# pymc-devs/nutpie

Measured on AMD Instinct MI355X. Metric: leapfrog steps/sec (all chains), higher is better.
Workload: dtype f64

## Files before the change

### include/nutpie_hip.h

```cpp
#ifndef NUTPIE_HIP_H
#define NUTPIE_HIP_H

#include <stdint.h>

#ifdef __cplusplus
extern "C" {
#endif

#define NPHIP_OK 0
#define NPHIP_ERR (-1)
#define NPHIP_ERR_UNKNOWN_ATTR (-2)
#define NPHIP_ERR_NOT_AVAILABLE (-3)
#define NPHIP_ERR_BAD_VALUE (-4)

#define NPHIP_WAIT_DONE 0
#define NPHIP_WAIT_TIMEOUT 1
#define NPHIP_WAIT_ERROR 2

const char* nphip_last_error(void);
const char* nphip_version(void);
int nphip_device_count(void);

typedef struct nphip_settings nphip_settings_t;

// ... 39 lines not shown

typedef struct nphip_sampler nphip_sampler_t;

typedef struct {
    uint64_t finished_draws;
    uint64_t total_draws;
    uint64_t divergences;
    int32_t tuning;
    int32_t started;
    uint64_t latest_num_steps;
    uint64_t total_num_steps;
    double step_size;
    uint64_t runtime_ms;
} nphip_chain_progress_t;

typedef struct {
    int32_t device;
    int32_t waves_per_chain;
    uint64_t chain_offset;
    uint64_t n_local_chains;
    void* stream;
    int32_t store_draws;
    int32_t evals_per_launch;
    int32_t start_paused;
    int32_t manual;
    void* staging_q;
    void* staging_grad;
    void* staging_logp;
    int32_t no_register_kernel;
    int32_t no_stream_cache;
    int32_t graph_steps;
    int32_t host_groups;
    int32_t host_persist;
    int32_t reserved_;
} nphip_launch_t;

void nphip_launch_defaults(nphip_launch_t*);
int nphip_default_evals_per_launch(uint64_t dim);
uint64_t nphip_abi_struct_size(int which );

nphip_sampler_t* nphip_sampler_create(const nphip_settings_t*, const nphip_model_t*, const nphip_launch_t*);
void nphip_sampler_free(nphip_sampler_t*);
int nphip_sampler_wait(nphip_sampler_t*, int64_t timeout_ms);
int nphip_sampler_step(nphip_sampler_t*, uint64_t n_launches, double* kernel_ms, uint64_t* launches_done);
int nphip_sampler_pause(nphip_sampler_t*);
int nphip_sampler_resume(nphip_sampler_t*);
int nphip_sampler_abort(nphip_sampler_t*);
int nphip_sampler_is_finished(nphip_sampler_t*);
int nphip_sampler_progress(nphip_sampler_t*, uint64_t local_chain, nphip_chain_progress_t* out);
int nphip_sampler_waves_per_chain(const nphip_sampler_t*);
uint64_t nphip_sampler_num_chains(const nphip_sampler_t*);
uint64_t nphip_sampler_dim(const nphip_sampler_t*);
uint64_t nphip_sampler_total_draws(const nphip_sampler_t*);
double nphip_sampler_seconds(const nphip_sampler_t*);
uint64_t nphip_sampler_launches(const nphip_sampler_t*);
enum { NPHIP_HOST_MODE_NONE = 0, NPHIP_HOST_MODE_LAUNCH_PER_EVALUATION = 1, NPHIP_HOST_MODE_GROUPS = 2, NPHIP_HOST_MODE_RESIDENT = 3,
       NPHIP_HOST_MODE_FELL_BACK = 4 };
int nphip_sampler_host_mode(const nphip_sampler_t* s);

int nphip_sampler_finished_draws(nphip_sampler_t*, uint64_t* finished);
int nphip_sampler_copy_stat(nphip_sampler_t*, const char* name, void* host_out, uint64_t nbytes);
int nphip_sampler_copy_expanded(nphip_sampler_t*, void* host_out, uint64_t nbytes);
int64_t nphip_sampler_waiting(nphip_sampler_t*, uint8_t* mask);
int nphip_sampler_resume_at(nphip_sampler_t*, uint64_t n, const uint64_t* local_chains, const double* positions, int on_device);
int nphip_sampler_set_metric(nphip_sampler_t*, uint64_t n, const uint64_t* local_chains, uint64_t k, const double* sigma2, const double* V,
                             const double* lambda, int on_device);
int nphip_sampler_stage_metric(nphip_sampler_t*, uint64_t n, const uint64_t* local_chains, uint64_t k, const double* sigma2, const double* V,
// ... 28 lines not shown
```

### nutpie_amd/_lib.py

```python

from __future__ import annotations

import ctypes as C
import json
import os
import subprocess
import threading

import numpy as np

_HERE = os.path.dirname(os.path.abspath(__file__))
_LIB_PATH = os.environ.get("NUTPIE_HIP_LIB") or os.path.join(_HERE, "libnutpie_hip.so")
_CSRC = os.path.join(_HERE, "csrc")

__version__ = "0.1.0"

NPHIP_OK = 0
NPHIP_ERR_UNKNOWN_ATTR = -2
NPHIP_ERR_NOT_AVAILABLE = -3
NPHIP_ERR_BAD_VALUE = -4
WAIT_DONE, WAIT_TIMEOUT, WAIT_ERROR = 0, 1, 2

RAW_LOGP_FN = C.CFUNCTYPE(C.c_int, C.c_uint64, C.POINTER(C.c_double), C.POINTER(C.c_double), C.POINTER(C.c_double), C.c_void_p)
RAW_EXPAND_FN = C.CFUNCTYPE(C.c_int, C.c_uint64, C.c_uint64, C.POINTER(C.c_double), C.POINTER(C.c_double), C.c_void_p)
DEVICE_EXPAND_FN = C.CFUNCTYPE(C.c_int, C.c_uint64, C.c_uint64, C.c_uint64, C.c_void_p, C.c_void_p, C.c_void_p, C.c_void_p)
DEVICE_LOGP_FN = C.CFUNCTYPE(C.c_int, C.c_uint64, C.c_uint64, C.c_void_p, C.c_void_p, C.c_void_p, C.c_void_p, C.c_void_p)


class _Launch(C.Structure):
    _fields_ = [
        ("device", C.c_int32),
        ("waves_per_chain", C.c_int32),
        ("chain_offset", C.c_uint64),
        ("n_local_chains", C.c_uint64),
        ("stream", C.c_void_p),
        ("store_draws", C.c_int32),
        ("evals_per_launch", C.c_int32),
        ("start_paused", C.c_int32),
        ("manual", C.c_int32),
        ("staging_q", C.c_void_p),
        ("staging_grad", C.c_void_p),
        ("staging_logp", C.c_void_p),
        ("no_register_kernel", C.c_int32),
        ("no_stream_cache", C.c_int32),
        ("graph_steps", C.c_int32),
        ("host_groups", C.c_int32),
        ("host_persist", C.c_int32),
        ("reserved_", C.c_int32),
    ]


class _Progress(C.Structure):
    _fields_ = [
        ("finished_draws", C.c_uint64),
        ("total_draws", C.c_uint64),
        ("divergences", C.c_uint64),
        ("tuning", C.c_int32),
        ("started", C.c_int32),
        ("latest_num_steps", C.c_uint64),
        ("total_num_steps", C.c_uint64),
        ("step_size", C.c_double),
        ("runtime_ms", C.c_uint64),
    ]


_lib = None
_lib_lock = threading.Lock()


def build(force: bool = False) -> str:
    srcs = [os.path.join(_CSRC, f) for f in ("kernels.hip", "host.hip", "linalg.hip", "lowrank_est.hip", "engine_types.h", "kernel_families.h", "dense_tile.h", "Makefile")]
    srcs += [os.path.join(_HERE, "..", "include", f) for f in ("nutpie_hip.h", "nphip_spec.h")]
    stale = not os.path.exists(_LIB_PATH) or os.path.getmtime(_LIB_PATH) < max(os.path.getmtime(s) for s in srcs)
    if force or stale:
        r = subprocess.run(["make", "-j", str(max(1, min(8, os.cpu_count() or 1))), "-C", _CSRC] + (["-B"] if force else []), capture_output=True, text=True)
        if r.returncode != 0:
            raise RuntimeError("building libnutpie_hip.so failed:\n" + r.stdout + r.stderr)
    return _LIB_PATH


def lib():
# ... 469 lines not shown

_STAT_DTYPES = {
    "depth": np.int64, "n_steps": np.int64, "index_in_trajectory": np.int64,
    "diverging": np.bool_, "maxdepth_reached": np.bool_, "tuning": np.bool_,
    "energy": np.float64, "energy_error": np.float64, "logp": np.float64, "step_size": np.float64,
    "step_size_bar": np.float64, "mean_tree_accept": np.float64, "mean_tree_accept_sym": np.float64,
}
_VECTOR_STATS = ("gradient", "mass_matrix_inv", "divergence_start", "divergence_end", "divergence_momentum", "divergence_start_gradient")


class PyTrace:

    def __init__(self, draws, stats, finished, chain_offset=0, expanded=None):
        self.draws = draws
        self.stats = stats
        self.finished = finished
        self.chain_offset = chain_offset
        self.expanded = expanded

    def is_arrow(self):
        return False

    def is_zarr(self):
        return False

    def is_dense(self):
        return True


class PySampler:

    def __init__(self, settings: PyNutsSettings, model: _Model, *, device=0, waves_per_chain=0, chain_offset=0,
                 n_local_chains=0, stream=None, store_draws=True, evals_per_launch=0, start_paused=False, manual=False,
                 staging=None, no_register_kernel=False, no_stream_cache=False, graph_steps=0, host_groups=0, host_persist=None):
        L = lib()
        la = _Launch()
        L.nphip_launch_defaults(C.byref(la))
        la.device = int(device)
        la.waves_per_chain = int(waves_per_chain)
        la.chain_offset = int(chain_offset)
        la.n_local_chains = int(n_local_chains)
        la.stream = C.c_void_p(stream) if stream else None
        la.store_draws = int(bool(store_draws))
        la.evals_per_launch = int(evals_per_launch)
        la.start_paused = int(bool(start_paused))
        la.manual = int(bool(manual))
        la.no_register_kernel = int(bool(no_register_kernel))
        la.no_stream_cache = int(bool(no_stream_cache))
        la.graph_steps = int(graph_steps)
        la.host_groups = int(host_groups)
        if host_persist is None:
            host_persist = 1 if getattr(model, "_python_callable", False) else 0
        la.host_persist = int(host_persist)
        if staging is not None:
            la.staging_q, la.staging_grad, la.staging_logp = (C.c_void_p(int(p)) for p in staging)
        self._model = model
        self._settings = settings
        self._chain_offset = int(chain_offset)
        self._store_draws = bool(store_draws)
        h = L.nphip_sampler_create(settings._h, model._h, C.byref(la))
        if not h:
            raise RuntimeError(_err())
        self._h = C.c_void_p(h)
        self._results = None

    @classmethod
    def from_pyfunc(cls, settings, cores, model, progress_type=None, extra_callback=None, extra_callback_rate=None, store=None, **kw):
        if store is not None:
            raise NotImplementedError("storage back-ends (zarr / arrow) are outside the scope of the HIP engine: the trace lives in HBM")
        if progress_type is not None or extra_callback is not None:
            raise NotImplementedError("progress templates / callbacks are handled by nutpie_amd.sample(), not by the sampler handle")
        return cls(settings, model, **kw)

    from_pymc = from_pyfunc
    from_stan = from_pyfunc

    def _require(self):
        if self._h is None:
            raise RuntimeError("Sampler is empty (results were taken)")

    @property
# ... 333 lines not shown
```

### nutpie_amd/csrc/engine_types.h

```cpp
#pragma once

#include <stdint.h>

namespace nphip {

constexpr int kMaxDepthCap = 16;
constexpr int kLrMax = 16;

enum Phase : int64_t {
    PH_START = 0,
    PH_INIT_EVAL = 1,
    PH_SS_FIRST = 2,
    PH_SS_ITER = 3,
    PH_TREE = 4,
    PH_DONE = 5,
    PH_ERROR = 6,
    PH_WAIT_HOST = 7,
    PH_RESUME_SS = 8,
    PH_DRAW_END = 9,
    PH_DRAW_BEGIN = 10,
};

enum ChainError : int64_t {
    CE_NONE = 0,
// ... 79 lines not shown
struct Args {
    DevSettings s;
    int64_t n_chains;
    int64_t chain_offset;
    int64_t dim, ld;
    int32_t cap;
    int32_t npslots, nqpool;
    Ctl* ctl;
    double* qpool;
    double* pslots;
    double* sig2;
    double* est;
    const double* m_mu;
    const double* m_a;
    const double* m_b;
    const double* m_bsh;
    double* qeval;
    double* geval;
    double* ueval;
    int64_t* ecode;
    const double* init_points;
    double* tr_draws;
    double* tr_grad;
    double* tr_mm;
    double* tr_div[4];
    int64_t* st_depth; int64_t* st_nsteps; int64_t* st_idx;
    uint8_t* st_diverging; uint8_t* st_maxdepth; uint8_t* st_tuning;
    double* st_energy; double* st_energy_error; double* st_logp; double* st_step; double* st_step_bar;
    double* st_accept; double* st_accept_sym;
    int32_t reg_nv;
    int32_t stream_cache;
    int32_t sig_lds;
    int32_t lean;
    int32_t max_evals;
    int32_t have_result;
    unsigned long long* counters;
    unsigned int* grp_arrive;
    volatile unsigned long long* grp_flag;
    volatile unsigned long long* grp_go;
    unsigned long long* grp_go_dev;
    int32_t pvec;
    int32_t lr_on;
    float* lr_V;
    double* lr_lam;
    double* lr_std;
    double* st_sig2;
    float* st_V;
    double* st_lam;
    const void* dens_data;
    int32_t dens_lds_doubles;
    int32_t dens_shared_doubles;
    const double* dg_P;
    const double* dg_mu;
    int64_t dg_KP;
    unsigned long long* dg_sync;
    int32_t dg_variant, dg_pad_;
};
constexpr int kDgSyncWords = 128 * 32 + 16 + 16 + 8 * 256 / 2;
constexpr unsigned long long kGoLast = 1ull << 32;
constexpr unsigned long long kGoSeqMask = 0xffffffffull;
constexpr unsigned long long kPubAllDone = 1ull << 62, kPubError = 1ull << 63;
constexpr unsigned long long kRollGo = 1, kRollFail = 2;

struct LaunchSlice {
    int chain_lo, chain_n;
    int grp;
// ... 10 lines not shown
```

### nutpie_amd/csrc/host.hip

```cpp
#include <hip/hip_runtime.h>
#include <sched.h>

#include <algorithm>
#include <atomic>
#include <chrono>
#include <cmath>
#include <condition_variable>
#include <cstdio>
#include <cstring>
#include <functional>
#include <memory>
#include <map>
#include <mutex>
#include <string>
#include <thread>
#include <vector>

#include "../../include/nutpie_hip.h"
#include "../../include/nphip_spec.h"
#include "engine_types.h"
#include "kernel_families.h"

namespace nphip {
hipError_t launch_advance(const Args& a, const Args* d_args, bool fused, int W, hipStream_t st, const LaunchSlice* slice = nullptr);
// ... 811 lines not shown
    s.early_mm_switch_freq = (int64_t)set.early_mass_matrix_switch_freq;
    s.mm_update_freq = (int64_t)set.mass_matrix_update_freq;
    s.initial_step = set.initial_step; s.target_accept = set.target_accept;
    s.jitter = set.jitter; s.max_step_size = set.max_step_size;
    s.adapt_adam = set.adam ? 1 : 0; s.adam_lr = set.adam_learning_rate;
    s.da_k = set.da_k; s.da_t0 = set.da_t0; s.da_gamma = set.da_gamma;
    s.init_kind = model.init_kind; s.num_try_init = (int32_t)set.num_try_init;
    s.store_draws = launch.store_draws; s.store_gradient = set.store_gradient;
    s.store_mass_matrix = set.store_mass_matrix; s.store_divergences = set.store_divergences;
    if (!set.pause_draws.empty()) {
        if (!launch.manual) { set_error("pause draws need a manual-mode sampler (launch.manual = 1): the caller resumes the chains"); return false; }
        for (uint64_t pd : set.pause_draws)
            if (pd == 0 || pd >= set.num_tune) { set_error("pause draws must lie inside the warm-up (0 < draw < num_tune)"); return false; }
    }
    s.n_pause = (int32_t)set.pause_draws.size();
    for (size_t i = 0; i < set.pause_draws.size(); ++i) s.pause_draws[i] = (int64_t)set.pause_draws[i];

    args.n_chains = (int64_t)n;
    args.chain_offset = (int64_t)launch.chain_offset;
    args.dim = (int64_t)dim;
    args.ld = geo.ld;
    args.cap = (int32_t)set.maxdepth;
    args.npslots = num_pslots(args.cap);
    args.nqpool = num_qpool(args.cap);
    const size_t ld = (size_t)args.ld;
    args.reg_nv = geo.reg_nv;
    args.lean = geo.lean ? 1 : 0;
    args.stream_cache = geo.stream_cache ? 1 : 0;
    args.pvec = lrm ? 3 : 2;
    args.lr_on = lrm ? 1 : 0;
    s.low_rank_metric = lrm ? 1 : 0;

    args.sig_lds = geo.sig_lds ? 1 : 0;

    if (!dalloc(&args.ctl, n)) return false;
    if (!dalloc(&args.qpool, n * args.nqpool * 2 * ld)) return false;
    if (!dalloc(&args.pslots, n * args.npslots * (size_t)args.pvec * ld)) return false;
    if (lrm && (!dalloc(&args.lr_V, n * (size_t)kLrMax * ld) || !dalloc(&args.lr_lam, n * (size_t)kLrMax) || !dalloc(&args.lr_std, n * ld))) return false;
    if (lrm && (!dalloc(&args.st_V, n * (size_t)kLrMax * ld) || !dalloc(&args.st_lam, n * (size_t)kLrMax) || !dalloc(&args.st_sig2, n * ld))) return false;
    if (!dalloc(&args.sig2, n * ld)) return false;
    if (!dalloc(&args.est, n * 8 * ld)) return false;
    if (!dalloc(&args.counters, 4)) return false;
    if (fused) {
        double *mu = nullptr, *a = nullptr, *b = nullptr;
        if (!dalloc(&mu, ld) || !dalloc(&a, ld) || !dalloc(&b, ld)) return false;
        HIP_TRY(hipMemcpyAsync(mu, model.mu.data(), dim * 8, hipMemcpyHostToDevice, stream));
        HIP_TRY(hipMemcpyAsync(a, model.a.data(), dim * 8, hipMemcpyHostToDevice, stream));
        bpad.assign(ld, -0.0);
        std::copy(model.b.begin(), model.b.begin() + (dim > 0 ? dim - 1 : 0), bpad.begin());
        HIP_TRY(hipMemcpyAsync(b, bpad.data(), ld * 8, hipMemcpyHostToDevice, stream));
        args.m_mu = mu; args.m_a = a; args.m_b = b;
        double* bsh = nullptr;
        if (!dalloc(&bsh, ld + 8)) return false;
        bshpad.assign(ld + 8, -0.0);
        std::copy(model.b.begin(), model.b.begin() + (dim > 0 ? dim - 1 : 0), bshpad.begin() + 1);
        HIP_TRY(hipMemcpyAsync(bsh, bshpad.data(), (ld + 8) * 8, hipMemcpyHostToDevice, stream));
        args.m_bsh = bsh;
    } else {
        const uint64_t zc_limit = (n <= 1024 && dim <= 1024) ? (8u << 20) : (4u << 20);
        zero_copy = (model.kind == 1) && !(launch.staging_q && launch.staging_grad && launch.staging_logp) && n * dim * 8 <= zc_limit;
        if (launch.staging_q && launch.staging_grad && launch.staging_logp) {
            args.qeval = (double*)launch.staging_q; args.geval = (double*)launch.staging_grad; args.ueval = (double*)launch.staging_logp;
        } else if (!zero_copy && (!dalloc(&args.qeval, n * dim) || !dalloc(&args.geval, n * dim) || !dalloc(&args.ueval, n))) return false;
        if (dens) {
            args.dens_data = model.jit_data;
            args.dens_lds_doubles = (int32_t)(model.jit_lds_bytes / 8);
// ... 1269 lines not shown
```

### nutpie_amd/csrc/kernel_families.h

```cpp
#pragma once
#include <cstddef>
#include <cstdint>
#include <type_traits>
#include <utility>

#ifndef NPHIP_W1_OCC2_MAX
#ifdef NPHIP_JIT_DENSITY
#define NPHIP_W1_OCC2_MAX 0
#else
#define NPHIP_W1_OCC2_MAX 3
#endif
#endif
#ifndef NPHIP_RW_OCC2_MAX
#define NPHIP_RW_OCC2_MAX 4
#endif
#ifndef NPHIP_CB_OCC
#define NPHIP_CB_OCC(W) 2
#endif
#ifndef NPHIP_LEAN_OCC
#define NPHIP_LEAN_OCC(W) ((W) <= 4 ? 1 : ((W) <= 8 ? 2 : 4))
#endif

namespace nphip {

// ... 2 lines not shown

enum class DynLds : int {
    none,
    sigma2,
    sigma2_and_summary,
    sigma2_if_staged
};

struct KernelFamily {
    Family family;
    bool fused, lean, remote, lr, wide, denseg;
    int waves;
    int nv_lo, nv_hi;
    int part;
    DynLds dyn;
};

inline constexpr KernelFamily kW1One         = {Family::w1,             true,  false, false, false, false, false, 1,                  1, 1,   0,    DynLds::none};
inline constexpr KernelFamily kW1            = {Family::w1,             true,  false, false, false, false, false, 1,                  2, 8,   12,   DynLds::none};
inline constexpr KernelFamily kW1Wide        = {Family::w1_wide,        true,  false, false, false, true,  false, 1,                  2, 3,   12,   DynLds::none};
inline constexpr KernelFamily kW1Lr          = {Family::w1_lr,          true,  false, false, true,  false, false, 1,                  1, 8,   8,    DynLds::none};
inline constexpr KernelFamily kRing          = {Family::ring,           true,  false, false, false, false, false, 2 | 4,              1, 8,   3,    DynLds::none};
inline constexpr KernelFamily kRingLr        = {Family::ring_lr,        true,  false, false, true,  false, false, 2 | 4,              5, 8,   9,    DynLds::none};
inline constexpr KernelFamily kLean4         = {Family::lean,           true,  true,  false, false, false, false, 4,                  9, 24,  1,    DynLds::sigma2_and_summary};
inline constexpr KernelFamily kLean8         = {Family::lean,           true,  true,  false, false, false, false, 8,                  1, 10,  2,    DynLds::sigma2};
inline constexpr KernelFamily kMemory        = {Family::memory,         true,  false, false, false, false, false, 1 | 2 | 4 | 8 | 16, -1, 0,  4,    DynLds::sigma2_if_staged};
inline constexpr KernelFamily kMemoryCached  = {Family::memory,         true,  false, false, false, false, false, 1,                  -8, -8, 4,    DynLds::none};
inline constexpr KernelFamily kRemoteW1      = {Family::remote,         false, false, true,  false, false, false, 1,                  1, 8,   5,    DynLds::none};
inline constexpr KernelFamily kRemoteWn      = {Family::remote,         false, false, true,  false, false, false, 2 | 4,              1, 8,   6,    DynLds::none};
inline constexpr KernelFamily kDenseResident = {Family::dense_resident, false, false, true,  false, false, true,  1,                  1, 8,   11,   DynLds::none};

inline constexpr KernelFamily kFamilies[] = {kW1One, kW1, kW1Wide, kW1Lr, kRing, kRingLr, kLean4, kLean8, kMemory, kMemoryCached, kRemoteW1, kRemoteWn, kDenseResident};

inline constexpr int kWideMaxChains = 1024;
inline constexpr int kMemoryWaves = 8;
inline constexpr int kMaxWaves = 16;

constexpr bool has(const KernelFamily& f, int W, int64_t nv) { return W > 0 && (f.waves & W) == W && (W & (W - 1)) == 0 && nv >= f.nv_lo && nv <= f.nv_hi; }
constexpr int chains_per_group(int W) { return W == 1 ? 4 : 1; }
constexpr int group_threads(int W) { return 64 * W * chains_per_group(W); }

inline constexpr int kLdsBytes = 160 * 1024, kChunkBytes = 128 * 8;
constexpr int lean_free_chunks(int W, int nv) { return W == 4 ? (kLdsBytes - (nv > 20 ? 12288 : 8192) - nv * W * kChunkBytes) / (W * kChunkBytes) : 0; }

constexpr size_t dyn_lds_bytes(const KernelFamily& f, int W, int nv, int64_t ld, bool sig_lds) {
    const size_t sigma2 = (size_t)ld * 8;
    const int free_chunks = lean_free_chunks(W, nv), summary = free_chunks < 0 ? 0 : (free_chunks < 2 * nv ? free_chunks : 2 * nv);
    return f.dyn == DynLds::sigma2 ? sigma2
         : f.dyn == DynLds::sigma2_and_summary ? sigma2 + (size_t)summary * (size_t)(W * kChunkBytes)
         : (f.dyn == DynLds::sigma2_if_staged && W >= 8 && sig_lds) ? sigma2 : 0;
}

constexpr bool two_waves_per_simd(int W, int NV, bool LR, bool WIDE) { return NV > 0 && !LR && !WIDE && NV <= (W == 1 ? NPHIP_W1_OCC2_MAX : NPHIP_RW_OCC2_MAX); }
template <bool FUSED, int W, int NV, bool LEAN, bool REMOTE, bool LR, bool WIDE>
constexpr int min_waves() { return LEAN ? NPHIP_LEAN_OCC(W) : (two_waves_per_simd(W, NV, LR, WIDE) ? 2 : ((!FUSED && NV == 0 && !REMOTE) ? NPHIP_CB_OCC(W) : 1)); }
template <bool FUSED, int W, int NV, bool LEAN, bool REMOTE, bool LR, bool WIDE>
constexpr int max_waves() { return LEAN ? NPHIP_LEAN_OCC(W) : (two_waves_per_simd(W, NV, LR, WIDE) ? 2 : 8); }

#ifdef NPHIP_ONLY_FAMILY
#ifndef NPHIP_ONLY_W
#define NPHIP_ONLY_W 0
#endif
#ifndef NPHIP_ONLY_NV
#define NPHIP_ONLY_NV -1000
#endif
constexpr bool built(const KernelFamily& f, int W, int nv) {
// ... 15 lines not shown
```

### nutpie_amd/csrc/kernels.hip

```cpp
#include <hip/hip_runtime.h>

#include "../../include/nphip_spec.h"
#include "engine_types.h"
#include "kernel_families.h"

#if defined(__HIP_DEVICE_COMPILE__)
#define NPHIP_GLOBAL __attribute__((address_space(1)))
#define NPHIP_LDS __attribute__((address_space(3)))
#define NPHIP_CONST __attribute__((address_space(4)))
#else
#define NPHIP_GLOBAL
#define NPHIP_LDS
#define NPHIP_CONST
#endif

#ifdef NPHIP_JIT_DENSITY
#define NPHIP_JIT 1
#else
#define NPHIP_JIT 0
#endif

namespace nphip {


// ... 1808 lines not shown
    __device__ __forceinline__ void issue_leaf_hot(Hot& H) const {
        const int32_t j = H.nleaf + 1, d = H.depth;
        int32_t newp;
        if (j == (1 << d)) newp = H.end_newp;
        else if (j & 1) newp = (j == 1) ? slot_first(d) : slot_first(__builtin_ctz((unsigned)(j - 1)));
        else newp = slot_last(__builtin_ctz((unsigned)j), A.cap);
        H.newq = (int32_t)__builtin_ctz(~(H.used_base | H.sub_used | (1u << H.srcq)));
        H.newp = newp;
    }
    __device__ __forceinline__ void start_doubling_hot(Hot& H) const {
        nphip_u32x4 r = nphip_philox(A.s.seed, (uint32_t)H.depth, gchain, H.draw, NPHIP_RNG_DIRECTION);
        H.dir = (r.v[0] & 1u) ? 1 : -1;
        const int db = H.dir > 0 ? 1 : 0;
        H.nleaf = 0;
        H.srcq = rfl(c->endq[db]);
        H.srcp = rfl(c->endp[db]);
        H.idx_cur = rfl(H.dir > 0 ? c->idx_right : c->idx_left);
        H.sub_used = 0u;
        hot_doubling(H);
        issue_leaf_hot(H);
    }
    __device__ __forceinline__ double merge_uniform_hot(const Hot& H, int32_t j, int32_t d, int32_t k, nphip_u32x4& blk, int32_t& blk_id) const {
        const int32_t id = k >> 1;
        if (blk_id != id) {
            const uint32_t c3 = (uint32_t)NPHIP_RNG_MERGE | ((uint32_t)d << 8) | ((uint32_t)id << 16);
            blk = nphip_philox(A.s.seed, (uint32_t)j, gchain, H.draw, c3);
            blk_id = id;
        }
        return (k & 1) ? nphip_u01(blk.v[2], blk.v[3]) : nphip_u01(blk.v[0], blk.v[1]);
    }

    __device__ __forceinline__ void merge_level(Hot& H, int32_t j, int32_t d, int32_t k, nphip_u32x4& blk, int32_t& blk_id, double& T_wm, int64_t& T_we,
                                                int32_t& T_q, double& T_U, double& T_E, int32_t& T_idx) {
        double sm; int64_t se;
        const int32_t A_q = rfl(c->sub_q[k]), A_idx = rfl(c->sub_idx[k]);
        const double A_U = c->sub_U[k], A_E = c->sub_E[k];
        H.sub_used &= ~(1u << A_q);
        nphip_w_add(c->sub_wm[k], c->sub_we[k], T_wm, T_we, &sm, &se);
        const bool take = merge_uniform_hot(H, j, d, k, blk, blk_id) * sm < nphip_w_rel(T_wm, T_we, se);
        if (!take) { T_q = A_q; T_U = A_U; T_E = A_E; T_idx = A_idx; }
        T_wm = sm; T_we = se;
    }

    __device__ __forceinline__ bool leaf_reg(RegsT& X, Hot& H, int32_t& end_code_out) {
        constexpr int nk = NVX;
        const int32_t j = H.nleaf + 1, d = H.depth, dir = H.dir;
        const int db = dir > 0 ? 1 : 0;
        const int32_t idx_new = H.idx_cur + dir;
        const int32_t srcq = H.srcq, srcp = H.srcp, newq = H.newq, newp = H.newp;
        const bool check = H.check;
#ifdef NPHIP_PROFILE
        const int64_t tp0 = (int64_t)__builtin_readcyclecounter();
#endif
        if (X.reg_q != srcq) {
            const double* q = Q(srcq);
#pragma unroll
            for (int k = 0; k < NVX; ++k) if (k < nk) X.q[k] = ld2(q, ridx(k));
            if (REMOTE) {
                const double* g = G(srcq);
#pragma unroll
                for (int k = 0; k < NVX; ++k) if (k < nk) X.g[k] = ld2(g, ridx(k));
            } else {
                regs_grad(X);
            }
        }
        if (X.reg_p != srcp) { load_slot(srcp, X.p, X.r); if (LR) load_slot_v(srcp, X.v); }
        if (!X.sig_ok) {
#pragma unroll
            for (int k = 0; k < NVX; ++k) if (k < nk) X.s[k] = ld2(sig2, ridx(k));
            if (LR) {
                const double* sdp = A.lr_std + (size_t)chain * ld;
#pragma unroll
                for (int k = 0; k < NVX; ++k) X.sd[k] = ld2(sdp, ridx(k));
            }
            X.sig_ok = true;
        }
        if (j == 1) { X.ring_leaf0 = -1; X.ring_leaf1 = -1; }
        const bool lrm = LR && lr_job() && rfl(c->host_metric) != 0;
// ... 139 lines not shown
            lr_dispatch(lrk, [&](auto kc) {
#pragma unroll
                for (int k = 0; k < NVX; ++k) {
                    double2 u;
                    u.x = X.sd[k].x * X.p[k].x; u.y = X.sd[k].y * X.p[k].y;
                    const double2 w = lr_apply_c<decltype(kc)::value>(ridx(k), u, lrc);
                    X.v[k].x = X.sd[k].x * w.x; X.v[k].y = X.sd[k].y * w.y;
                }
            });
#pragma unroll
            for (int k = 0; k < NVX; ++k) {
                accK.x = fma(X.p[k].x, X.v[k].x, accK.x);
                accK.y = fma(X.p[k].y, X.v[k].y, accK.y);
                const double tx0 = (X.r[k].x - rold[k].x) + pold[k].x, ty0 = (X.r[k].y - rold[k].y) + pold[k].y;
                accE.x = fma(tx0, X.v[k].x, accE.x);
                accE.y = fma(ty0, X.v[k].y, accE.y);
                accS.x = fma(tx0, vold[k].x, accS.x);
                accS.y = fma(ty0, vold[k].y, accS.y);
            }
        }
        X.reg_q = newq;
        X.reg_p = newp;
        X.dirty_qg = true;
        X.dirty_pr = true;
        if (!LR && !NORING) {
            if ((j & 3) == 1) { ring_write(0, X.p, X.r); X.ring_leaf0 = j; }
            else if ((j & 3) == 2) { ring_write(1, X.p, X.r); X.ring_leaf1 = j; }
        }
#ifdef NPHIP_PROFILE
        const int64_t tp1 = (int64_t)__builtin_readcyclecounter();
#endif
        NPHIP_PHASE_FENCE();
        double v4[4] = {accK.x + accK.y, accL.x + accL.y, accE.x + accE.y, accS.x + accS.y};
        rsum(v4);
        NPHIP_PHASE_FENCE();
#ifdef NPHIP_PROFILE
        const int64_t tp2 = (int64_t)__builtin_readcyclecounter();
        c->prof[0] += tp1 - tp0; c->prof[6] += tp2 - tp1;
#endif
        const double K = 0.5 * v4[0], lp = (REMOTE && !DG) ? lp_remote : 0.5 * v4[1];
        const bool turn0 = (v4[2] < 0.0) || (v4[3] < 0.0);
        if (REMOTE && code_remote < 0) { X.dirty_qg = X.dirty_pr = false; hot_save(H); finish_chain(PH_ERROR, CE_FATAL_LOGP); return true; }
        H.nleaf += 1;
        H.n_steps += 1;
        const bool ok = isfinite(lp) && (!REMOTE || code_remote == 0);
        const double Unew = -lp, E = K + Unew, dE = E - H.H0;
        const bool diverged = !ok || (dE > H.max_ee) || !isfinite(dE);
        double T_wm = 1.0;
        int64_t T_we = 0;
        nphip_u32x4 mrg_blk = {{0u, 0u, 0u, 0u}};
        int32_t mrg_id = -1;
        {
            if (!diverged) {
                const double x = -dE, xc = x > 1e9 ? 1e9 : (x < -1e9 ? -1e9 : x);
                double kk;
                nphip_exp_parts(xc, &T_wm, &kk);
                T_we = (int64_t)kk;
                const double e = nphip_exp_scale(x, T_wm, kk);
                const double a = e < 1.0 ? e : 1.0;
                H.acc += a;
                H.acc_sym += 2.0 * a / (1.0 + e);
            }
        }
        if (diverged) { X.dirty_qg = X.dirty_pr = false; hot_save(H);
            if (ENDOUT) end_code_out = end_code(true, false, FUSED, ok, !REMOTE, FUSED); else rare_end_draw(A, c, red, chain, true, false, FUSED, ok, !REMOTE, FUSED);
            return true; }
#ifdef NPHIP_PROFILE
        int64_t tq = (int64_t)__builtin_readcyclecounter();
        c->prof[8] += tq - tp2;
#endif

        NPHIP_PHASE_FENCE();
        double T_U = Unew, T_E = E;
        int32_t T_q = newq, T_idx = idx_new;
        H.srcq = newq; H.srcp = newp; H.idx_cur = idx_new;
        double2 obp[NVX], obr[NVX], obv[NVX];
        int32_t k = 0;
        while (k < d && (((j - 1) >> k) & 1)) {
            if (check) {
                bool turn;
                if (k == 0) {
                    turn = turn0;
                } else if (LR) {
                    const int32_t a = j - (2 << k) + 1, al = j - (1 << k);
                    load_slot(first_slot_of(a, d), obp, obr); load_slot_v(first_slot_of(a, d), obv);
// ... 3 lines not shown
#pragma unroll
                        for (int q_ = 0; q_ < NVX; ++q_) { pold[q_] = obp[q_]; rold[q_] = obr[q_]; vold[q_] = obv[q_]; }
                    }
                    if (!turn) {
                        const int32_t sl_ = slot_last(__builtin_ctz((unsigned)al), A.cap);
                        load_slot(sl_, obp, obr); load_slot_v(sl_, obv);
                        turn = sub_b_v(X, obp, obr, obv);
                    }
                } else {
                    const int32_t a = j - (2 << k) + 1, al = j - (1 << k);
                    if (k == 1 && X.ring_leaf0 == a) ring_read(0, obp, obr);
                    else load_slot(first_slot_of(a, d), obp, obr);
                    if (k == 2) {
                        if (X.ring_leaf0 == al + 1) ring_read(0, pold, rold);
                        else load_slot(first_slot_of(al + 1, d), pold, rold);
                    }
                    turn = sub_a(X, obp, obr, pold, rold);
                    if (k >= 2) {
#pragma unroll
                        for (int q_ = 0; q_ < NVX; ++q_) { pold[q_] = obp[q_]; rold[q_] = obr[q_]; }
                    }
                    if (!turn) {
                        if (k == 1 && X.ring_leaf1 == al) ring_read(1, obp, obr);
                        else load_slot(slot_last(__builtin_ctz((unsigned)al), A.cap), obp, obr);
                        turn = sub_b(X, obp, obr);
                    }
                }
                if (turn) { X.dirty_qg = X.dirty_pr = false; hot_save(H); if (ENDOUT) end_code_out = end_code(false, false, false, false, !REMOTE, false); else rare_end_draw(A, c, red, chain, false, false, false, false, !REMOTE); return true; }
            }
#ifdef NPHIP_PROFILE
            { const int64_t t_ = (int64_t)__builtin_readcyclecounter(); c->prof[k == 0 ? 9 : 10] += t_ - tq; tq = t_; }
#endif
            NPHIP_PHASE_FENCE();
            merge_level(H, j, d, k, mrg_blk, mrg_id, T_wm, T_we, T_q, T_U, T_E, T_idx);
            NPHIP_PHASE_FENCE();
#ifdef NPHIP_PROFILE
            { const int64_t t_ = (int64_t)__builtin_readcyclecounter(); c->prof[11] += t_ - tq; tq = t_; }
#endif
            ++k;
        }
        if (k < d) {
            c->sub_wm[k] = T_wm; c->sub_we[k] = T_we; c->sub_q[k] = T_q; c->sub_U[k] = T_U; c->sub_E[k] = T_E; c->sub_idx[k] = T_idx;
            H.sub_used |= 1u << T_q;
#ifdef NPHIP_PROFILE
            const int64_t tp3 = (int64_t)__builtin_readcyclecounter();
#endif
            store_state(X, T_q == newq, LR || NORING || ((j & 3) == 0) || ((j & 7) == 1));
            issue_leaf_hot(H);
#ifdef NPHIP_PROFILE
            c->prof[7] += (int64_t)__builtin_readcyclecounter() - tp3;
#endif
            return false;
        }
        bool turn = false;
        if (check) {
            const int32_t far_slot = rfl(c->endp[1 - db]), far_idx = rfl(dir > 0 ? c->idx_left : c->idx_right);
            const int32_t near_idx = rfl(dir > 0 ? c->idx_right : c->idx_left);
            if (d == 0) {
                turn = LR ? check1_v(X, pold, pold, vold, far_idx, idx_new) : check1(X, pold, pold, far_idx, idx_new);
            } else if (LR) {
                if (d == 2) { load_slot(slot_first((int)d), pold, rold); load_slot_v(slot_first((int)d), vold); }
                load_slot(far_slot, obp, obr); load_slot_v(far_slot, obv);
                turn = check_a_v(X, obp, obr, obv, pold, rold, vold, far_idx, near_idx + dir, idx_new);
                if (!turn) {
                    load_slot(rfl(c->endp[db]), obp, obr); load_slot_v(rfl(c->endp[db]), obv);
                    turn = check1_v(X, obp, obr, obv, near_idx, idx_new);
                }
// ... 1202 lines not shown
                    if (budget <= 0) break;
                    --budget;
                } else {
                    if (!have) break;
                    have = false;
                }
            }
            worked = true;
            if (ph != PH_TREE) {
                rare_phase_fn(A, c, red, chain, ph);
                continue;
            }
            RegsT X;
            SCacheT Y;
            Hot H;
            constexpr bool HOT = NV > 0;
            if (HOT) hot_load(H);
            int32_t end_code_ = 0;
            bool rare = false, out_of_budget = false;
            int lean_end = 0;
            const LeanRs lrs = lean_rs();
            if ((NV == 0 || NV == -1 || LEAN) && sig_copy != nullptr) {
                for (int64_t i = 2 * (int64_t)threadIdx.x; i < ld; i += 2 * (int64_t)blockDim.x)
                    *(NPHIP_LDS double2*)(sig_copy + i) = ld2(sig2, i);
                __syncthreads();
                sig_lds = sig_copy;
            }
            for (;;) {
#ifdef NPHIP_PROFILE
                const int64_t t0 = (int64_t)__builtin_readcyclecounter();
#endif
                if (NV > 0) {
                    if (LEAN) { lean_end = leaf_lean(lrs, X, H); rare = lean_end != 0; }
                    else rare = leaf_reg(X, H, end_code_);
                } else {
                    double lp = 0.0;
                    int64_t code = 0;
                    if (FUSED && !lr_job()) {
                        bool turn0 = false;
                        const bool even_leaf = ((c->nleaf + 1) & 1) == 0;
                        const double K = lf_stream(lp, c->idx_cur + c->dir, turn0, Y);
                        rare = cont_tree(X, Y, K, lp, code, even_leaf, turn0);
                    } else {
                        if (FUSED) lf1(c->lf_srcq, c->lf_srcp, c->lf_newq, c->lf_newp, c->lf_sign);
                        CbCrit cr;
                        bool fast = false;
                        if (cb_fast_ok()) {
                            lp = A.ueval[chain];
                            code = A.ecode ? A.ecode[chain] : 0;
                            fast = code == 0 && isfinite(lp);
                        }
                        const double K = fast ? leaf_cb(cr) : lf2(lp, code, c->idx_cur + c->dir);
#ifdef NPHIP_PROFILE
                        c->prof[0] += (int64_t)__builtin_readcyclecounter() - t0;
#endif
                        rare = cont_tree(X, Y, K, lp, code, false, false, fast ? &cr : nullptr);
                    }
                }
#ifdef NPHIP_PROFILE
                const int64_t t2 = (int64_t)__builtin_readcyclecounter();
                c->prof[3] += 1;
                if (rare) { c->prof[2] += t2 - t0; c->prof[5] += 1; } else { c->prof[1] += t2 - t0; c->prof[4] += 1; }
#endif
                if (rare || (!HOT && c->phase != PH_TREE)) break;
                if (REMOTE && !DENS && !DG) {
                    if (c->hs_last != 0) { out_of_budget = true; break; }
                } else if (FUSED || DENS || DG) {
// ... 619 lines not shown
```

### profiles/make_traffic.py

```python
import json
import os
import re

HERE = os.path.dirname(os.path.abspath(__file__))
SOURCES = {
    "1000:1": ("r6_d1000_timed_config_pmc.txt", 1024 * 2048, "k_advance<fused,W=1,NV=8>",
               "bench.py default: sampling phase, positions stored, 2048 leapfrogs per chain per launch; the timed launches"),
    "2000:2": ("r1_d2000_multiwave_kernel_pmc.txt", 1024 * 128, "k_advance<fused,W=2,NV=8>", "round 1: tuning phase, 128 leapfrogs per chain per launch"),
    "10000:4": ("r5_d10000_timed_config_pmc.txt", 1024 * 512, "k_advance<fused,W=4,NV=20,lean>",
                "bench.py --dim 10000: sampling phase, positions stored, 512 leapfrogs per chain per launch; the timed launches"),
}
JOBS = {
    "config3_compiled_density": ("r6_config3_compiled_density_final_pmc.txt", "k_advance<callback,W=1,NV=2,REMOTE> of the generated radon density (512 chains, tune 400 + draws 1000)"),
    "config3_traced_torch_density": ("r6_config3_traced_torch_density_final_pmc.txt", "the same model traced from its torch log-density (nutpie_amd.torch_trace)"),
    "low_rank_173_k4": ("r5_low_rank_d173_k4_pmc.txt", "k_advance<fused,W=1,NV=2,LR>: AR(1) Gaussian D = 173, 512 chains, 4 columns handed in; the launches after the hand-in"),
    "config2ii_dense_resident": ("r6_dense_resident_pmc.txt", "k_advance<callback,W=1,NV=8,REMOTE,DENSEG>: the dense 1000-dim Gaussian's resident kernel (launch-wide fp64 MFMA GEMM inside the leaf), 1024 chains; 12 launches of 256 evaluation rounds in the sampling phase (scratch/r6_dense_job.py)"),
    "low_rank_1000_k16": ("r5_low_rank_d1000_k16_pmc.txt", "k_advance<fused,W=1,NV=8,LR>: AR(1) Gaussian D = 1000, 1024 chains, 16 columns handed in; the launches after the hand-in"),
}
FALLBACK = {
    "1000:1": ("r2_d1000_kernel_pmc.txt", 1024 * 256, "round 2: tuning phase, 256 leapfrogs per chain per launch"),
    "10000:4": ("r2_d10000_lean_lds_slot_e128_pmc.txt", 1024 * 128, "round 2: tuning phase, 128 leapfrogs per chain per launch"),
}


def counter(txt, name):
    m = re.search(name + r"\s+n=\s*\d+\s+mean=([0-9.e+]+)", txt)
    return float(m.group(1)) if m else None


def main():
    out = {}
    for key, (fn, lpl, kernel, config) in SOURCES.items():
        if not os.path.exists(os.path.join(HERE, fn)) and key in FALLBACK:
            fn, lpl, config = FALLBACK[key]
        txt = open(os.path.join(HERE, fn)).read()
        f, w = counter(txt, "FETCH_SIZE"), counter(txt, "WRITE_SIZE")
        e = {"bytes_per_leapfrog": (2 * f + w) * 1024 / lpl, "leapfrogs_per_launch": lpl, "kernel": kernel, "source": "profiles/" + fn,
             "config": config, "fetch_size_kb": f, "write_size_kb": w}
        insts = {k: counter(txt, "SQ_INSTS_" + k.upper()) for k in ("valu", "salu", "lds", "vmem_rd", "vmem_wr")}
# ... 40 lines not shown
```

Baseline: 240.2 million.

## Fuse pairs of leapfrog leaves into one reduction and acceptance pass

Adds a paired-leaf path for single-wave fused kernels with small NV. The first leaf's leapfrog is run inline and its kinetic and log-density partial sums ride along in the second leaf's cross-lane reduction. The two acceptance exponentials are computed in the two wave halves, and the first leaf is merged as a tree record without a separate leaf iteration. This is meant to halve reduction and sync overhead per leaf. It costs register pressure and extra rollback logic when the first leaf diverges. It can be disabled with a new launch flag.

```diff
diff --git a/include/nutpie_hip.h b/include/nutpie_hip.h
--- a/include/nutpie_hip.h
+++ b/include/nutpie_hip.h
@@ -95,7 +95,7 @@
     int32_t graph_steps;
     int32_t host_groups;
     int32_t host_persist;
-    int32_t reserved_;
+    int32_t no_leaf_pairs;
 } nphip_launch_t;
 
 void nphip_launch_defaults(nphip_launch_t*);
diff --git a/nutpie_amd/_lib.py b/nutpie_amd/_lib.py
--- a/nutpie_amd/_lib.py
+++ b/nutpie_amd/_lib.py
@@ -46,7 +46,7 @@
         ("graph_steps", C.c_int32),
         ("host_groups", C.c_int32),
         ("host_persist", C.c_int32),
-        ("reserved_", C.c_int32),
+        ("no_leaf_pairs", C.c_int32),
     ]
 
 
@@ -582,7 +582,8 @@
 
     def __init__(self, settings: PyNutsSettings, model: _Model, *, device=0, waves_per_chain=0, chain_offset=0,
                  n_local_chains=0, stream=None, store_draws=True, evals_per_launch=0, start_paused=False, manual=False,
-                 staging=None, no_register_kernel=False, no_stream_cache=False, graph_steps=0, host_groups=0, host_persist=None):
+                 staging=None, no_register_kernel=False, no_stream_cache=False, graph_steps=0, host_groups=0, host_persist=None,
+                 no_leaf_pairs=False):
         L = lib()
         la = _Launch()
         L.nphip_launch_defaults(C.byref(la))
@@ -597,6 +598,7 @@
         la.manual = int(bool(manual))
         la.no_register_kernel = int(bool(no_register_kernel))
         la.no_stream_cache = int(bool(no_stream_cache))
+        la.no_leaf_pairs = int(bool(no_leaf_pairs))
         la.graph_steps = int(graph_steps)
         la.host_groups = int(host_groups)
         if host_persist is None:
diff --git a/nutpie_amd/csrc/engine_types.h b/nutpie_amd/csrc/engine_types.h
--- a/nutpie_amd/csrc/engine_types.h
+++ b/nutpie_amd/csrc/engine_types.h
@@ -135,6 +135,7 @@
     int32_t stream_cache;
     int32_t sig_lds;
     int32_t lean;
+    int32_t no_leaf_pairs;
     int32_t max_evals;
     int32_t have_result;
     unsigned long long* counters;
diff --git a/nutpie_amd/csrc/host.hip b/nutpie_amd/csrc/host.hip
--- a/nutpie_amd/csrc/host.hip
+++ b/nutpie_amd/csrc/host.hip
@@ -867,6 +867,7 @@
     s.low_rank_metric = lrm ? 1 : 0;
 
     args.sig_lds = geo.sig_lds ? 1 : 0;
+    args.no_leaf_pairs = launch.no_leaf_pairs != 0 ? 1 : 0;
 
     if (!dalloc(&args.ctl, n)) return false;
     if (!dalloc(&args.qpool, n * args.nqpool * 2 * ld)) return false;
diff --git a/nutpie_amd/csrc/kernel_families.h b/nutpie_amd/csrc/kernel_families.h
--- a/nutpie_amd/csrc/kernel_families.h
+++ b/nutpie_amd/csrc/kernel_families.h
@@ -58,6 +58,11 @@
 
 inline constexpr KernelFamily kFamilies[] = {kW1One, kW1, kW1Wide, kW1Lr, kRing, kRingLr, kLean4, kLean8, kMemory, kMemoryCached, kRemoteW1, kRemoteWn, kDenseResident};
 
+#ifndef NPHIP_LEAF_PAIRS_NV_MASK
+#define NPHIP_LEAF_PAIRS_NV_MASK 0x1FC
+#endif
+constexpr bool leaf_pairs(int W, int NV) { return W == 1 && NV >= 2 && NV <= 8 && ((NPHIP_LEAF_PAIRS_NV_MASK >> NV) & 1) != 0; }
+
 inline constexpr int kWideMaxChains = 1024;
 inline constexpr int kMemoryWaves = 8;
 inline constexpr int kMaxWaves = 16;
diff --git a/nutpie_amd/csrc/kernels.hip b/nutpie_amd/csrc/kernels.hip
--- a/nutpie_amd/csrc/kernels.hip
+++ b/nutpie_amd/csrc/kernels.hip
@@ -1864,18 +1864,124 @@
 
     __device__ __forceinline__ void merge_level(Hot& H, int32_t j, int32_t d, int32_t k, nphip_u32x4& blk, int32_t& blk_id, double& T_wm, int64_t& T_we,
                                                 int32_t& T_q, double& T_U, double& T_E, int32_t& T_idx) {
-        double sm; int64_t se;
         const int32_t A_q = rfl(c->sub_q[k]), A_idx = rfl(c->sub_idx[k]);
         const double A_U = c->sub_U[k], A_E = c->sub_E[k];
+        merge_record(H, j, d, k, blk, blk_id, A_q, A_idx, A_U, A_E, c->sub_wm[k], c->sub_we[k], T_wm, T_we, T_q, T_U, T_E, T_idx);
+    }
+    __device__ __forceinline__ void merge_record(Hot& H, int32_t j, int32_t d, int32_t k, nphip_u32x4& blk, int32_t& blk_id, int32_t A_q, int32_t A_idx,
+                                                 double A_U, double A_E, double A_wm, int64_t A_we, double& T_wm, int64_t& T_we,
+                                                 int32_t& T_q, double& T_U, double& T_E, int32_t& T_idx) {
+        double sm; int64_t se;
         H.sub_used &= ~(1u << A_q);
-        nphip_w_add(c->sub_wm[k], c->sub_we[k], T_wm, T_we, &sm, &se);
+        nphip_w_add(A_wm, A_we, T_wm, T_we, &sm, &se);
         const bool take = merge_uniform_hot(H, j, d, k, blk, blk_id) * sm < nphip_w_rel(T_wm, T_we, se);
         if (!take) { T_q = A_q; T_U = A_U; T_E = A_E; T_idx = A_idx; }
         T_wm = sm; T_we = se;
     }
 
-    __device__ __forceinline__ bool leaf_reg(RegsT& X, Hot& H, int32_t& end_code_out) {
+    static constexpr bool PAIRS = FUSED && !LEAN && !REMOTE && !LR && !NORING && nphip::leaf_pairs(W, NV);
+    struct PairA {
+        int32_t nleaf, idx_cur, srcq, srcp, newq, newp;
+        uint32_t sub_used;
+        double accK, accL;
+    };
+    __device__ __forceinline__ void pair_first(RegsT& X, Hot& H, PairA& a) {
         constexpr int nk = NVX;
+        const int32_t j = H.nleaf + 1, dir = H.dir, idx_new = H.idx_cur + dir;
+        a.nleaf = H.nleaf; a.idx_cur = H.idx_cur; a.srcq = H.srcq; a.srcp = H.srcp; a.newq = H.newq; a.newp = H.newp; a.sub_used = H.sub_used;
+#ifdef NPHIP_PROFILE
+        const int64_t tp0 = (int64_t)__builtin_readcyclecounter();
+#endif
+        if (X.reg_q != H.srcq) {
+            const double* q = Q(H.srcq);
+#pragma unroll
+            for (int k = 0; k < NVX; ++k) if (k < nk) X.q[k] = ld2(q, ridx(k));
+            regs_grad(X);
+        }
+        if (X.reg_p != H.srcp) load_slot(H.srcp, X.p, X.r);
+        if (!X.sig_ok) {
+#pragma unroll
+            for (int k = 0; k < NVX; ++k) if (k < nk) X.s[k] = ld2(sig2, ridx(k));
+            X.sig_ok = true;
+        }
+        if (j == 1) { X.ring_leaf0 = -1; X.ring_leaf1 = -1; }
+        NPHIP_PHASE_FENCE();
+        const double eps = (double)dir * H.step;
+        const double h = 0.5 * eps;
+        if (idx_new == -1) {
+#pragma unroll
+            for (int k = 0; k < NVX; ++k) if (k < nk) { X.r[k].x = -0.0; X.r[k].y = -0.0; }
+        }
+        double2 z[NVX];
+#pragma unroll
+        for (int k = 0; k < NVX; ++k) if (k < nk) {
+            X.p[k].x = fma(h, X.g[k].x, X.p[k].x);
+            X.p[k].y = fma(h, X.g[k].y, X.p[k].y);
+            X.q[k].x = fma(eps, X.s[k].x * X.p[k].x, X.q[k].x);
+            X.q[k].y = fma(eps, X.s[k].y * X.p[k].y, X.q[k].y);
+            const double2 mu = par_mu(ridx(k));
+            z[k].x = X.q[k].x - mu.x;
+            z[k].y = X.q[k].y - mu.y;
+        }
+        publish_edges(z);
+        double2 accK = {0.0, 0.0}, accL = {0.0, 0.0};
+#pragma unroll
+        for (int k = 0; k < NVX; ++k) if (k < nk) {
+            double2 aa, b01, gg;
+            double b2, edge_zl, edge_zr;
+            par_ab(ridx(k), aa, b01, b2);
+            edge_pair(z, k, edge_zl, edge_zr);
+            const double zl = wave_shr1(z[k].y, edge_zl);
+            const double zr = wave_shl1(z[k].x, edge_zr);
+            double tx = aa.x * z[k].x;
+            tx = fma(b01.x, zl, tx);
+            tx = fma(b01.y, z[k].y, tx);
+            double ty = aa.y * z[k].y;
+            ty = fma(b01.y, z[k].x, ty);
+            ty = fma(b2, zr, ty);
+            gg.x = -tx;
+            gg.y = -ty;
+            accL.x = fma(z[k].x, gg.x, accL.x);
+            accL.y = fma(z[k].y, gg.y, accL.y);
+            X.g[k] = gg;
+            X.p[k].x = fma(h, gg.x, X.p[k].x);
+            X.p[k].y = fma(h, gg.y, X.p[k].y);
+            X.r[k].x = X.r[k].x + X.p[k].x;
+            X.r[k].y = X.r[k].y + X.p[k].y;
+            accK.x = fma(X.p[k].x, X.s[k].x * X.p[k].x, accK.x);
+            accK.y = fma(X.p[k].y, X.s[k].y * X.p[k].y, accK.y);
+        }
+        a.accK = accK.x + accK.y;
+        a.accL = accL.x + accL.y;
+        X.reg_q = H.newq;
+        X.reg_p = H.newp;
+        X.dirty_qg = true;
+        X.dirty_pr = true;
+        if ((j & 3) == 1) { ring_write(0, X.p, X.r); X.ring_leaf0 = j; }
+        store_state(X, true, (j & 7) == 1);
+        H.nleaf = j;
+        H.n_steps += 1;
+        H.srcq = a.newq; H.srcp = a.newp; H.idx_cur = idx_new;
+        H.sub_used |= 1u << a.newq;
+        issue_leaf_hot(H);
+#ifdef NPHIP_PROFILE
+        c->prof[0] += (int64_t)__builtin_readcyclecounter() - tp0;
+#endif
+    }
+    static __device__ __forceinline__ double exp_scale_select(double x, double p, double k) {
+        const int ki = (int)k;
+        const int k1 = ki / 2, k2 = ki - k1;
+        double e = (p * nphip_pow2i(k1)) * nphip_pow2i(k2);
+        e = x < -745.2 ? 0.0 : e;
+        e = x > 709.782712893384 ? (double)INFINITY : e;
+        return e;
+    }
+
+    __device__ __forceinline__ bool leaf_reg(RegsT& X, Hot& H, int32_t& end_code_out, const bool pair_ = false, bool* a_ended = nullptr) {
+        constexpr int nk = NVX;
+        const bool PAIR = PAIRS && pair_;
+        PairA pa = {};
+        if (PAIR) { pair_first(X, H, pa); NPHIP_PHASE_FENCE(); }
         const int32_t j = H.nleaf + 1, d = H.depth, dir = H.dir;
         const int db = dir > 0 ? 1 : 0;
         const int32_t idx_new = H.idx_cur + dir;
@@ -2081,7 +2187,14 @@
 #endif
         NPHIP_PHASE_FENCE();
         double v4[4] = {accK.x + accK.y, accL.x + accL.y, accE.x + accE.y, accS.x + accS.y};
-        rsum(v4);
+        double vA[2] = {0.0, 0.0};
+        if (PAIR) {
+            double v8[8] = {v4[0], v4[1], v4[2], v4[3], pa.accK, pa.accL, 0.0, 0.0};
+            rsum(v8);
+            v4[0] = v8[0]; v4[1] = v8[1]; v4[2] = v8[2]; v4[3] = v8[3]; vA[0] = v8[4]; vA[1] = v8[5];
+        } else {
+            rsum(v4);
+        }
         NPHIP_PHASE_FENCE();
 #ifdef NPHIP_PROFILE
         const int64_t tp2 = (int64_t)__builtin_readcyclecounter();
@@ -2090,6 +2203,19 @@
         const double K = 0.5 * v4[0], lp = (REMOTE && !DG) ? lp_remote : 0.5 * v4[1];
         const bool turn0 = (v4[2] < 0.0) || (v4[3] < 0.0);
         if (REMOTE && code_remote < 0) { X.dirty_qg = X.dirty_pr = false; hot_save(H); finish_chain(PH_ERROR, CE_FATAL_LOGP); return true; }
+        double A_U = 0.0, A_E = 0.0, A_dE = 0.0;
+        if (PAIR) {
+            const double K_A = 0.5 * vA[0], lp_A = 0.5 * vA[1];
+            const bool ok_A = isfinite(lp_A);
+            A_U = -lp_A; A_E = K_A + A_U; A_dE = A_E - H.H0;
+            if (!ok_A || (A_dE > H.max_ee) || !isfinite(A_dE)) {
+                H.idx_cur = pa.idx_cur; H.srcq = pa.srcq; H.srcp = pa.srcp; H.newq = pa.newq; H.newp = pa.newp; H.sub_used = pa.sub_used;
+                X.dirty_qg = X.dirty_pr = false; hot_save(H);
+                end_code_out = end_code(true, false, FUSED, ok_A, !REMOTE, FUSED);
+                *a_ended = true;
+                return true;
+            }
+        }
         H.nleaf += 1;
         H.n_steps += 1;
         const bool ok = isfinite(lp) && (!REMOTE || code_remote == 0);
@@ -2099,7 +2225,30 @@
         int64_t T_we = 0;
         nphip_u32x4 mrg_blk = {{0u, 0u, 0u, 0u}};
         int32_t mrg_id = -1;
-        {
+        double A_wm = 1.0;
+        int64_t A_we = 0;
+        if constexpr (PAIRS) {
+            if (PAIR || !diverged) {
+            const double x = lane < 32 ? -A_dE : -dE, xc = x > 1e9 ? 1e9 : (x < -1e9 ? -1e9 : x);
+            double wm, kk;
+            nphip_exp_parts(xc, &wm, &kk);
+            const double e = exp_scale_select(x, wm, kk);
+            const double a = e < 1.0 ? e : 1.0;
+            const double sym = 2.0 * a / (1.0 + e);
+            if (PAIR) {
+                A_wm = readlane_f64(wm, 0);
+                A_we = (int64_t)readlane_f64(kk, 0);
+                H.acc += readlane_f64(a, 0);
+                H.acc_sym += readlane_f64(sym, 0);
+            }
+            if (!diverged) {
+                T_wm = readlane_f64(wm, 32);
+                T_we = (int64_t)readlane_f64(kk, 32);
+                H.acc += readlane_f64(a, 32);
+                H.acc_sym += readlane_f64(sym, 32);
+            }
+            }
+        } else {
             if (!diverged) {
                 const double x = -dE, xc = x > 1e9 ? 1e9 : (x < -1e9 ? -1e9 : x);
                 double kk;
@@ -2169,7 +2318,8 @@
             { const int64_t t_ = (int64_t)__builtin_readcyclecounter(); c->prof[k == 0 ? 9 : 10] += t_ - tq; tq = t_; }
 #endif
             NPHIP_PHASE_FENCE();
-            merge_level(H, j, d, k, mrg_blk, mrg_id, T_wm, T_we, T_q, T_U, T_E, T_idx);
+            if (PAIR && k == 0) merge_record(H, j, d, 0, mrg_blk, mrg_id, pa.newq, pa.idx_cur + dir, A_U, A_E, A_wm, A_we, T_wm, T_we, T_q, T_U, T_E, T_idx);
+            else merge_level(H, j, d, k, mrg_blk, mrg_id, T_wm, T_we, T_q, T_U, T_E, T_idx);
             NPHIP_PHASE_FENCE();
 #ifdef NPHIP_PROFILE
             { const int64_t t_ = (int64_t)__builtin_readcyclecounter(); c->prof[11] += t_ - tq; tq = t_; }
@@ -3438,7 +3588,17 @@
 #endif
                 if (NV > 0) {
                     if (LEAN) { lean_end = leaf_lean(lrs, X, H); rare = lean_end != 0; }
-                    else rare = leaf_reg(X, H, end_code_);
+                    else {
+                        bool pair = false;
+                        if constexpr (PAIRS) pair = (H.nleaf & 1) == 0 && H.depth >= 1 && budget >= 1 && A.no_leaf_pairs == 0;
+                        bool a_ended = false;
+                        if (pair) --budget;
+                        rare = leaf_reg(X, H, end_code_, pair, &a_ended);
+                        if (a_ended) ++budget;
+#ifdef NPHIP_PROFILE
+                        if (pair && !a_ended) { c->prof[3] += 1; c->prof[4] += 1; }
+#endif
+                    }
                 } else {
                     double lp = 0.0;
                     int64_t code = 0;
diff --git a/profiles/make_traffic.py b/profiles/make_traffic.py
--- a/profiles/make_traffic.py
+++ b/profiles/make_traffic.py
@@ -4,7 +4,7 @@
 
 HERE = os.path.dirname(os.path.abspath(__file__))
 SOURCES = {
-    "1000:1": ("r6_d1000_timed_config_pmc.txt", 1024 * 2048, "k_advance<fused,W=1,NV=8>",
+    "1000:1": ("leaf_pairs_d1000_timed_config_pmc.txt", 1024 * 2048, "k_advance<fused,W=1,NV=8>",
                "bench.py default: sampling phase, positions stored, 2048 leapfrogs per chain per launch; the timed launches"),
     "2000:2": ("r1_d2000_multiwave_kernel_pmc.txt", 1024 * 128, "k_advance<fused,W=2,NV=8>", "round 1: tuning phase, 128 leapfrogs per chain per launch"),
     "10000:4": ("r5_d10000_timed_config_pmc.txt", 1024 * 512, "k_advance<fused,W=4,NV=20,lean>",
```

Result: faster. 254.6 million, median of 6 (+6.0%).
